# zfountas/deep-active-inference-mc

Measured on AMD Instinct MI355X. Metric: EFE rollouts/sec (64x64 dSprites, 10 MC-samples, depth 5), higher is better.
Workload: dtype f32; 1 GPU; calculate_G_repeated: 128 rows (32 roots x 4 actions) x depth 5 x 10 MC samples per GPU (BASELINE configs[1]) + action posterior; rows_per_gpu=128, samples=10, depth=5, parallelism=episodes sharded x1, weights replicated

## Files before the change

### deep-active-inference-mc_amd/csrc/decoder.hip

```cpp
#include <utility>
#include "mfma_pipe.h"

namespace efe {

template <class F, int... I> __device__ __forceinline__ void static_for_(F&& f, std::integer_sequence<int, I...>) { (f(std::integral_constant<int, I>{}), ...); }
template <int N, class F> __device__ __forceinline__ void static_for(F&& f) { static_for_(f, std::make_integer_sequence<int, N>{}); }

__host__ __device__ constexpr int w3_nch(int G) { return G == 4 ? 5 : 4; }
__host__ __device__ constexpr int w3_prod(int G, int c) {
    return G < 4 ? 5 * ((G >> 1) + 2 * (c >> 1)) + (G & 1) + 2 * (c & 1)
         : G == 4 ? (c < 2 ? 5 * (1 + 2 * c) + 4 : c < 4 ? 20 + 1 + 2 * (c - 2) : 24)
                  : (c < 2 ? 5 * (2 * c) + 4 : 20 + 2 * (c - 2));
}
__host__ __device__ constexpr bool w3_direct(int pp) { return f22_o1(pp / 5) < 0 && f22_o1(pp % 5) < 0; }
__host__ __device__ constexpr int w3_view(int pp) { return 3 * f22_view(pp / 5) + f22_view(pp % 5); }
__host__ __device__ constexpr int w3_mat(int pp) { return 4 * f22_wt(pp / 5) + f22_wt(pp % 5); }
__host__ __device__ constexpr bool w3_hits(int pp, int o) {
    const int r = o >> 2, c = o & 3, pr = pp / 5, pc = pp % 5;
    return (r == f22_o0(pr) || r == f22_o1(pr)) && (c == f22_o0(pc) || c == f22_o1(pc));
}
__host__ __device__ constexpr bool w3_seen(int G, int c, int o) {
    for (int g = 0; g < G; ++g)
        for (int k = 0; k < w3_nch(g); ++k) if (w3_hits(w3_prod(g, k), o)) return true;
    if (!w3_direct(w3_prod(G, c)))
        for (int k = 0; k < w3_nch(G); ++k)
            if ((w3_direct(w3_prod(G, k)) || k < c) && w3_hits(w3_prod(G, k), o)) return true;
    return false;
}
__host__ __device__ constexpr bool w3_uses_view(int G, int vi) {
    for (int k = 0; k < w3_nch(G); ++k) if (w3_view(w3_prod(G, k)) == vi) return true;
    return false;
}
__host__ __device__ constexpr bool f22_in(int a, int r) { return a == 0 ? r <= 1 : (a == 1 ? r == 1 : r >= 1); }
__host__ __device__ constexpr bool w3_reads(int G, int r, int c) {
    for (int vi = 0; vi < 9; ++vi) if (w3_uses_view(G, vi) && f22_in(vi / 3, r) && f22_in(vi % 3, c)) return true;
    return false;
}

constexpr int DA_PS = 17;
constexpr int DA_BIAS = 273 * DA_PS;

__host__ __device__ constexpr int wino_i0(int a) { return a == 0 ? 0 : (a == 2 ? 2 : 1); }
__host__ __device__ constexpr int wino_i1(int a) { return a == 0 ? 2 : (a == 1 ? 2 : (a == 2 ? 1 : 3)); }
__host__ __device__ constexpr float wino_s1(int a) { return a == 1 ? 1.0f : -1.0f; }
__host__ __device__ constexpr float wino_at(int r, int a) { return r == 0 ? (a < 3 ? 1.0f : 0.0f) : (a == 0 ? 0.0f : (a == 1 ? 1.0f : -1.0f)); }

template <int NR, int R0, class Pix>
__device__ __forceinline__ void wino_l1(f32x16 (&out)[NR][2], const float4* __restrict__ U, const float4* sm, const int h,
                                        const int mt_, Pix pix) {
    constexpr int PD = 4;
    const unsigned ln = (threadIdx.x & 63u) * 16u;
    const __amdgpu_buffer_rsrc_t ur = wrsrc(U);
    int mt = mt_; asm volatile("" : "+s"(mt));
    constexpr int a_lo = NR == 2 ? 0 : R0, a_hi = NR == 2 ? 4 : R0 + 3;
    auto ufrag = [&](int a, int b, int kc) { return wfrag(ur, ln, (size_t)(((4 * a + b) * 2 + mt) * 8 + kc) * 64); };
    auto bases = [&](int a, int b, int (&pb)[4]) {
        const int i0 = wino_i0(a), i1 = wino_i1(a), j0 = wino_i0(b), j1 = wino_i1(b);
        pb[0] = pix(i0, j0); pb[1] = pix(i0, j1); pb[2] = pix(i1, j0); pb[3] = pix(i1, j1);
    };
    float4 aq[PD], raw[4];
    int pb[4];
#pragma unroll
    for (int p = 0; p < PD; ++p) aq[p] = ufrag(a_lo, 0, p);
    bases(a_lo, 0, pb);
#pragma unroll
    for (int q = 0; q < 4; ++q) raw[q] = sm[pb[q] + h];
    f32x16 xacc;
    const f32x16 zero = {};
    auto otrans = [&](int a, int b, const f32x16& m, auto mask) {
        constexpr int MASK = decltype(mask)::value;
#pragma unroll
        for (int r = 0; r < NR; ++r) {
            if (!((MASK >> r) & 1)) continue;
            const float car = wino_at(R0 + r, a);
#pragma unroll
            for (int c = 0; c < 2; ++c) {
                const float cbc = wino_at(c, b);
                if (cbc == 0.0f) continue;
                const float cf = car * cbc;
#pragma unroll
                for (int e = 0; e < 16; ++e) out[r][c][e] = __builtin_fmaf(cf, m[e], out[r][c][e]);
            }
        }
    };
    auto xi_row = [&](int a, auto mask) {
        const float s1 = wino_s1(a);
        const int an = a + 1 < a_hi ? a + 1 : a;
#pragma unroll
        for (int b = 0; b < 4; ++b) {
            const float t1 = wino_s1(b);
#pragma unroll
            for (int kc = 0; kc < 8; ++kc) {
                const float4 av = aq[kc % PD];
                aq[kc % PD] = (b * 8 + kc + PD < 32) ? ufrag(a, (b * 8 + kc + PD) >> 3, (kc + PD) & 7) : ufrag(an, 0, (kc + PD) & 7);
                float4 v;
                {
                    const float4 c0 = make_float4(__builtin_fmaf(s1, raw[2].x, raw[0].x), __builtin_fmaf(s1, raw[2].y, raw[0].y),
                                                  __builtin_fmaf(s1, raw[2].z, raw[0].z), __builtin_fmaf(s1, raw[2].w, raw[0].w));
                    const float4 c1 = make_float4(__builtin_fmaf(s1, raw[3].x, raw[1].x), __builtin_fmaf(s1, raw[3].y, raw[1].y),
                                                  __builtin_fmaf(s1, raw[3].z, raw[1].z), __builtin_fmaf(s1, raw[3].w, raw[1].w));
                    v = make_float4(__builtin_fmaf(t1, c1.x, c0.x), __builtin_fmaf(t1, c1.y, c0.y), __builtin_fmaf(t1, c1.z, c0.z), __builtin_fmaf(t1, c1.w, c0.w));
                }
                if (kc < 7) {
#pragma unroll
                    for (int q = 0; q < 4; ++q) raw[q] = sm[pb[q] + 2 * (kc + 1) + h];
                } else {
                    if (b < 3) bases(a, b + 1, pb);
                    else bases(an, 0, pb);
#pragma unroll
                    for (int q = 0; q < 4; ++q) raw[q] = sm[pb[q] + h];
                }
                __builtin_amdgcn_sched_barrier(0);
                f32x16& x = xacc;
                x = __builtin_amdgcn_mfma_f32_32x32x2f32(av.x, v.x, kc == 0 ? zero : x, 0, 0, 0);
                x = __builtin_amdgcn_mfma_f32_32x32x2f32(av.y, v.y, x, 0, 0, 0);
                x = __builtin_amdgcn_mfma_f32_32x32x2f32(av.z, v.z, x, 0, 0, 0);
                x = __builtin_amdgcn_mfma_f32_32x32x2f32(av.w, v.w, x, 0, 0, 0);
            }
            otrans(a, b, xacc, mask);
        }
    };
    if constexpr (NR == 2) {
        xi_row(0, std::integral_constant<int, 1>{});
#pragma unroll 1
        for (int a = 1; a < 3; ++a) xi_row(a, std::integral_constant<int, 3>{});
        xi_row(3, std::integral_constant<int, 2>{});
    } else {
#pragma unroll 1
        for (int a = a_lo; a < a_hi; ++a) xi_row(a, std::integral_constant<int, 1>{});
    }
}
struct F22Nb { int xb, c2[3], r2; };
__device__ __forceinline__ f32x4 f22_wfrag(const __amdgpu_buffer_rsrc_t wr, const unsigned ln, int ct, int m, int kc) {
    return __builtin_bit_cast(f32x4, wfrag(wr, ln + (unsigned)kc * 1024u, (size_t)(m * 4 + ct) * 256));
}
constexpr int F22_PD = 2;
__device__ __forceinline__ void f22_l2_first(f32x4 (&aq)[F22_PD][5], const __amdgpu_buffer_rsrc_t wr, const int dn, const unsigned ln) {
    static_for<F22_PD>([&](auto p) {
        static_for<w3_nch(p >> 2)>([&](auto c) { aq[p][c] = f22_wfrag(wr, ln, dn, w3_mat(w3_prod(p >> 2, c)), p & 3); });
    });
}
__device__ __forceinline__ void f22_l2(f32x4 (&acc)[16], f32x4 (&aq)[F22_PD][5], const __amdgpu_buffer_rsrc_t wr, const int dn,
                                       const unsigned ln, const f32x4 bias4, const f32x4* smv, const F22Nb& nb) {
    constexpr int NST = 24;
    auto px = [&](int i, int jj, int kc) -> f32x4 {
        return smv[(jj == 2 ? nb.c2[i] : (i == 2 ? nb.r2 + jj * DA_PS : nb.xb + (16 * i + jj) * DA_PS)) + 4 * kc];
    };
    auto view = [&](const f32x4 (&x)[9], int vi) -> f32x4 {
        const int va = vi / 3, vb = vi % 3;
        auto cv = [&](int i) -> f32x4 { return vb == 0 ? x[3 * i] - x[3 * i + 1] : (vb == 1 ? x[3 * i + 1] : x[3 * i + 2] - x[3 * i + 1]); };
        return va == 0 ? cv(0) - cv(1) : (va == 1 ? cv(1) : cv(2) - cv(1));
    };
    const f32x4 zero4 = {};
    f32x4 tq[5], xr[9];
    static_for<9>([&](auto i) { if constexpr (w3_reads(0, i / 3, i % 3)) xr[i] = px(i / 3, i % 3, 0); });
    static_for<NST>([&](auto stc) {
        constexpr int ST = decltype(stc)::value, G = ST >> 2, KC = ST & 3, GN = (ST + 1) >> 2, KN = (ST + 1) & 3;
        constexpr int SP = (ST + F22_PD) % NST, GP = SP >> 2, KP = SP & 3;
        f32x4 vw[9], ac[5];
        static_for<9>([&](auto vi) { if constexpr (w3_uses_view(G, vi)) vw[vi] = view(xr, vi); });
#pragma unroll
        for (int c = 0; c < 5; ++c) ac[c] = aq[ST % F22_PD][c];
        static_for<w3_nch(GP)>([&](auto c) { aq[ST % F22_PD][c] = f22_wfrag(wr, ln, ST + F22_PD < NST ? 0 : dn, w3_mat(w3_prod(GP, c)), KP); });
        if constexpr (ST + 1 < NST)
            static_for<9>([&](auto i) { if constexpr (w3_reads(GN, i / 3, i % 3)) xr[i] = px(i / 3, i % 3, KN); });
        __builtin_amdgcn_sched_barrier(0);
#pragma unroll
        for (int e = 0; e < 4; ++e)
            static_for<w3_nch(G)>([&](auto c) {
                constexpr int PP = w3_prod(G, c);
                const float b = vw[w3_view(PP)][e], av = ac[c][e];
                if constexpr (w3_direct(PP)) {
                    constexpr int O = 4 * f22_o0(PP / 5) + f22_o0(PP % 5);
                    constexpr bool FIRST = KC == 0 && !w3_seen(G, c, O);
                    acc[O] = __builtin_amdgcn_mfma_f32_16x16x4f32(av, b, (FIRST && e == 0) ? bias4 : acc[O], 0, 0, 0);
                } else {
                    tq[c] = __builtin_amdgcn_mfma_f32_16x16x4f32(av, b, (KC == 0 && e == 0) ? zero4 : tq[c], 0, 0, 0);
                }
            });
        if constexpr (KC == 3)
            static_for<w3_nch(G)>([&](auto c) {
                constexpr int PP = w3_prod(G, c);
                if constexpr (!w3_direct(PP))
                    static_for<16>([&](auto o) {
                        if constexpr (w3_hits(PP, o)) {
                            if constexpr (w3_seen(G, c, o)) acc[o] = acc[o] + tq[c];
                            else acc[o] = bias4 + tq[c];
                        }
                    });
            });
    });
}
__device__ __forceinline__ void f22_l2_store(f32x4 (&acc)[16], const __amdgpu_buffer_rsrc_t yr, const unsigned yoff, const int ct, const bool on) {
#pragma unroll
    for (int orow = 0; orow < 4; ++orow)
#pragma unroll
        for (int c = 0; c < 2; ++c) {
            u32x4 lo, hi;
#pragma unroll
            for (int e = 0; e < 4; ++e) {
                const unsigned x0 = __builtin_bit_cast(unsigned, relu_bits(acc[4 * orow + c][e]));
                const unsigned x1 = __builtin_bit_cast(unsigned, relu_bits(acc[4 * orow + c + 2][e]));
                const auto sw = __builtin_amdgcn_permlane32_swap(x0, x1, false, false);
                lo[e] = sw[0]; hi[e] = sw[1];
            }
            const unsigned so = (unsigned)(((2 * (orow & 1) + c) * 4096 + 2 * ct * 512 + (orow >> 1) * 32) * 16);
            if (on) {
                __builtin_amdgcn_raw_buffer_store_b128(lo, yr, yoff, so, 0);
                __builtin_amdgcn_raw_buffer_store_b128(hi, yr, yoff, so + 512u * 16u, 0);
            }
        }
}

__global__ void __launch_bounds__(256, 2) k_dec_a(const DecAArgs a) {
    constexpr int NTHR = 256;
    constexpr int NPH = 2048 / NTHR;
    constexpr int NPE = 8;
    extern __shared__ __attribute__((aligned(16))) float4 sm[];
    const int tid = threadIdx.x;
    const int lane = tid & 63;
    const int w = __builtin_amdgcn_readfirstlane(tid >> 6);

    const float4* W1 = reinterpret_cast<const float4*>(a.w1);
    const float4* W2 = reinterpret_cast<const float4*>(a.w2);

    if ((int)blockIdx.x >= a.rows) return;
    int* const slot = reinterpret_cast<int*>(sm + DA_BIAS + 32);
    if (tid == 0) slot[0] = 2 * (int)gridDim.x + atomicAdd(a.queue, 1);
    int nimg = (int)blockIdx.x + (int)gridDim.x;
    f32x4 pf[2 * NPH];
    f32x4* smv = reinterpret_cast<f32x4*>(sm);
    {
        const f32x4* X = reinterpret_cast<const f32x4*>(a.x4) + (size_t)blockIdx.x * 4096;
#pragma unroll
        for (int it = 0; it < 2 * NPH; ++it) pf[it] = X[w * 1024 + it * 64 + lane];
    }
    for (int i = tid; i < 17 * DA_PS; i += NTHR) sm[256 * DA_PS + i] = make_float4(0.f, 0.f, 0.f, 0.f);
    if (tid < 16) sm[DA_BIAS + tid] = reinterpret_cast<const float4*>(a.b1)[tid];
    else if (tid < 32) sm[DA_BIAS + tid] = reinterpret_cast<const float4*>(a.b2)[tid - 16];

    for (int img = blockIdx.x; img < a.rows;) {
        int tl_ = tid; asm volatile("" : "+v"(tl_));
        const int j = tl_ & 31, h = (tl_ >> 5) & 1;
        const bool live = row_live(a.live, img);
        if (live) {
            const int sbase = (64 * w + ((tl_ >> 4) & 3)) * DA_PS + (tl_ & 15);
#pragma unroll
            for (int it = 0; it < 2 * NPH; ++it) smv[sbase + it * 4 * DA_PS] = pf[it];
        }
        __syncthreads();
        const int nnimg = slot[0];
        int ticket = 0;
        if (tid == 0) ticket = 2 * (int)gridDim.x + atomicAdd(a.queue, 1);
        const int l1mt = w >> 1, l1n = 32 * (w & 1) + j;
        const int l1y = 2 * (l1n >> 3) - 1, l1x = 2 * (l1n & 7) - 1;
        if (live) {
            f32x16 l1o[2][2];
#pragma unroll
            for (int g4 = 0; g4 < 4; ++g4) {
                const float4 bb = sm[DA_BIAS + l1mt * 8 + 2 * g4 + h];
#pragma unroll
                for (int rc = 0; rc < 4; ++rc) { l1o[rc >> 1][rc & 1][4 * g4] = bb.x; l1o[rc >> 1][rc & 1][4 * g4 + 1] = bb.y; l1o[rc >> 1][rc & 1][4 * g4 + 2] = bb.z; l1o[rc >> 1][rc & 1][4 * g4 + 3] = bb.w; }
            }
            wino_l1<2, 0>(l1o, W1, sm, h, l1mt, [&](int i, int jj) {
                const int y = l1y + i, x = l1x + jj;
                return ((unsigned)y < 16u && (unsigned)x < 16u ? y * 16 + x : 256) * DA_PS;
            });
            __syncthreads();
            if (tid == 0) slot[0] = ticket;
#pragma unroll
            for (int rc = 0; rc < 4; ++rc) {
                const int pix = (l1y + 1 + (rc >> 1)) * 16 + l1x + 1 + (rc & 1);
#pragma unroll
                for (int g4 = 0; g4 < 4; ++g4) {
                    const f32x16& o = l1o[rc >> 1][rc & 1];
                    float4 v;
                    v.x = relu_bits(o[4 * g4 + 0]); v.y = relu_bits(o[4 * g4 + 1]);
                    v.z = relu_bits(o[4 * g4 + 2]); v.w = relu_bits(o[4 * g4 + 3]);
                    sm[pix * DA_PS + l1mt * 8 + 2 * g4 + h] = v;
                }
            }
        } else {
            __syncthreads();
            if (tid == 0) slot[0] = ticket;
        }
        __syncthreads();
        {
            int t2_ = tid; asm volatile("" : "+v"(t2_));
            const int n = t2_ & 15, g = (t2_ >> 4) & 3;
            const int bu = 2 * w + (n >> 3), bv = n & 7;
            const int zq = 256 * DA_PS + g;
            F22Nb nb;
            nb.xb = (32 * bu + 2 * bv) * DA_PS + g;
            nb.c2[0] = bv == 7 ? zq : nb.xb + 2 * DA_PS;
            nb.c2[1] = bv == 7 ? zq : nb.xb + 18 * DA_PS;
            nb.c2[2] = bv == 7 ? zq : nb.xb + 34 * DA_PS;
            nb.r2 = nb.xb + 32 * DA_PS;
            const unsigned ln = (unsigned)(t2_ & 63) * 16u;
            const unsigned yoff = (unsigned)(((32 * bu + 2 * bv + (g >> 1)) * 2 + (g & 1)) * 16);
            const __amdgpu_buffer_rsrc_t yr = wrsrc(a.y2 + (size_t)__builtin_amdgcn_readfirstlane(img) * (32 * 32 * 64));
            auto load_next = [&](const int lo, const int hi) {
                const int pimg = __builtin_amdgcn_readfirstlane(nimg < a.rows ? nimg : img);
                const __amdgpu_buffer_rsrc_t xr = wrsrc(a.x4 + (size_t)pimg * 16384);
#pragma unroll
                for (int it = 0; it < 2 * NPH; ++it)
                    if (it >= lo && it < hi) pf[it] = __builtin_bit_cast(f32x4, wfrag(xr, (unsigned)(w * 16384 + (t2_ & 63) * 16 + (it & 3) * 1024), (size_t)(it >> 2) * 256));
            };
            if (live) {
                f32x4 aq[F22_PD][5], acc2[16];
                f22_l2_first(aq, wrsrc(W2), 0, ln);
                load_next(0, NPE);
#pragma unroll 1
                for (int ct = 0; ct < 4; ++ct) {
                    const f32x4 bias4 = smv[DA_BIAS + 16 + 4 * ct + g];
                    f22_l2(acc2, aq, wrsrc(W2 + ct * 256), ct < 3 ? 1 : 0, ln, bias4, smv, nb);
                    if (ct < 3) f22_l2_store(acc2, yr, yoff, ct, true);
                }
                load_next(NPE, 2 * NPH);
                f22_l2_store(acc2, yr, yoff, 3, true);
            } else {
                load_next(0, 2 * NPH);
            }
        }
        __syncthreads();
        img = nimg; nimg = nnimg;
    }
}

constexpr int DAS_IN = 6 * 16;
constexpr int DAS_L1 = 4 * 16;
constexpr int DAS_BIAS = (DAS_IN + 1 + DAS_L1 + 2) * DA_PS;
constexpr size_t DAS_LDS_BYTES = (DAS_BIAS + 32) * sizeof(float4);
__global__ void __launch_bounds__(256, 2) k_dec_a_s(const DecAArgs a) {
    extern __shared__ __attribute__((aligned(16))) float4 sm[];
    float4* sin = sm;
    float4* sl1 = sm + (DAS_IN + 1) * DA_PS;
    const int tid = threadIdx.x, lane = tid & 63;
    const int w = __builtin_amdgcn_readfirstlane(tid >> 6);
    const int j = lane & 31, h = lane >> 5;
    const int img = blockIdx.x >> 3, p = blockIdx.x & 7;
    if (!row_live(a.live, img)) return;
    const float4* W1 = reinterpret_cast<const float4*>(a.w1);
    const float4* W2 = reinterpret_cast<const float4*>(a.w2);
    {
        const float4* X = reinterpret_cast<const float4*>(a.x4) + (size_t)img * 4096;
        const int c4 = tid & 15, px0 = tid >> 4;
        float4 v[6];
#pragma unroll
        for (int it = 0; it < 6; ++it) {
            const int pix = px0 + 16 * it, lr = pix >> 4, y = 2 * p - 1 + lr;
            v[it] = (y >= 0 && y < 16) ? X[(y * 16 + (pix & 15)) * 16 + c4] : make_float4(0.f, 0.f, 0.f, 0.f);
        }
#pragma unroll
        for (int it = 0; it < 6; ++it) sin[(px0 + 16 * it) * DA_PS + c4] = v[it];
    }
    if (tid < 16) sin[DAS_IN * DA_PS + tid] = make_float4(0.f, 0.f, 0.f, 0.f);
    if (tid < 2 * DA_PS) sl1[DAS_L1 * DA_PS + tid] = make_float4(0.f, 0.f, 0.f, 0.f);
    if (tid < 16) sm[DAS_BIAS + tid] = reinterpret_cast<const float4*>(a.b1)[tid];
    else if (tid < 32) sm[DAS_BIAS + tid] = reinterpret_cast<const float4*>(a.b2)[tid - 16];
    __syncthreads();
    const int mt = w >> 1;
    {
        const int r = w & 1, n = j & 15;
        const int ly = 2 * (n >> 3) - 1, lx = 2 * (n & 7) - 1;
        f32x16 o[1][2];
#pragma unroll
        for (int g4 = 0; g4 < 4; ++g4) {
            const float4 bb = sm[DAS_BIAS + mt * 8 + 2 * g4 + h];
#pragma unroll
            for (int c = 0; c < 2; ++c) { o[0][c][4 * g4] = bb.x; o[0][c][4 * g4 + 1] = bb.y; o[0][c][4 * g4 + 2] = bb.z; o[0][c][4 * g4 + 3] = bb.w; }
        }
        auto pix = [&](int i, int jj) {
            const int sy = ly + 1 + i, x = lx + jj, y = 2 * p - 1 + sy;
            return ((unsigned)y < 16u && (unsigned)x < 16u ? sy * 16 + x : DAS_IN) * DA_PS;
        };
        if (r) wino_l1<1, 1>(o, W1, sin, h, mt, pix);
        else wino_l1<1, 0>(o, W1, sin, h, mt, pix);
        if (j < 16)
#pragma unroll
        for (int c = 0; c < 2; ++c)
#pragma unroll
            for (int g4 = 0; g4 < 4; ++g4) {
                float4 v;
                v.x = relu_bits(o[0][c][4 * g4 + 0]); v.y = relu_bits(o[0][c][4 * g4 + 1]);
                v.z = relu_bits(o[0][c][4 * g4 + 2]); v.w = relu_bits(o[0][c][4 * g4 + 3]);
                sl1[((ly + 1 + r) * 16 + lx + 1 + c) * DA_PS + mt * 8 + 2 * g4 + h] = v;
            }
    }
    __syncthreads();
    {
        const int n = lane & 15, g = lane >> 4, bv = n & 7;
        const int zq = DAS_L1 * DA_PS + g;
        F22Nb nb;
        nb.xb = 2 * bv * DA_PS + g;
        nb.c2[0] = bv == 7 ? zq : nb.xb + 2 * DA_PS;
        nb.c2[1] = bv == 7 ? zq : nb.xb + 18 * DA_PS;
        nb.c2[2] = (bv == 7 || p == 7) ? zq : nb.xb + 34 * DA_PS;
        nb.r2 = p == 7 ? zq : nb.xb + 32 * DA_PS;
        const unsigned ln = (unsigned)lane * 16u;
        const unsigned yoff = (unsigned)(((32 * p + 2 * bv + (g >> 1)) * 2 + (g & 1)) * 16);
        const __amdgpu_buffer_rsrc_t yr = wrsrc(a.y2 + (size_t)img * (32 * 32 * 64));
        const __amdgpu_buffer_rsrc_t wr = wrsrc(W2 + w * 256);
        f32x4 aq[F22_PD][5], acc2[16];
        f22_l2_first(aq, wr, 0, ln);
        const f32x4 bias4 = reinterpret_cast<const f32x4*>(sm)[DAS_BIAS + 16 + 4 * w + g];
        f22_l2(acc2, aq, wr, 0, ln, bias4, reinterpret_cast<const f32x4*>(sl1), nb);
        f22_l2_store(acc2, yr, yoff, w, n < 8);
    }
}

constexpr size_t DA_LDS_BYTES = (DA_BIAS + 33) * sizeof(float4);
int init_dec_b_kernels();
int init_decoder_kernels() {
    if (hipFuncSetAttribute((const void*)k_dec_a, hipFuncAttributeMaxDynamicSharedMemorySize, DA_LDS_BYTES) != hipSuccess) return 1;
    if (hipFuncSetAttribute((const void*)k_dec_a_s, hipFuncAttributeMaxDynamicSharedMemorySize, DAS_LDS_BYTES) != hipSuccess) return 1;
    return init_dec_b_kernels();
}

void launch_dec_a(const DecAArgs& a, hipStream_t st) {
    if (a.parts == 8) {
        hipLaunchKernelGGL(k_dec_a_s, dim3(a.rows * 8), dim3(256), DAS_LDS_BYTES, st, a);
        return;
    }
    const size_t lds = DA_LDS_BYTES;
    const int grid = a.rows < 512 ? a.rows : 512;
    hipLaunchKernelGGL(k_dec_a, dim3(grid), dim3(256), lds, st, a);
}


template <int PARTS>
__global__ void __launch_bounds__(256, 2) k_dec_b4(const DecBArgs a) {
    constexpr int SR = 4, NW = 4, NTHR = 256;
    constexpr int DB_RP = 33;
    constexpr int DB_PS = 17;
    constexpr int DB_IN_F4 = (SR + 1) * DB_RP * DB_PS;
    constexpr int DB_YROWS = 4 * SR + 2;
    constexpr int NPF = (SR + 1) * 512 / NTHR;
    constexpr int NS = 32 / SR;
    constexpr int NST = 24;
    extern __shared__ __attribute__((aligned(16))) float4 sm[];
    float* sH = reinterpret_cast<float*>(sm + DB_IN_F4);
    __shared__ float4 sb3[8];
    const int tid = threadIdx.x;
    const int lane = tid & 63;
    const int w = __builtin_amdgcn_readfirstlane(tid >> 6);
    const int g = lane >> 4, v = lane & 15;
    const int u = w >> 1, hf = w & 1;
    constexpr int parts = PARTS;
    const int img = parts == 1 ? (int)blockIdx.x : (int)(blockIdx.x >> 2);
    const int qtr = parts == 1 ? 0 : (int)(blockIdx.x & 3);
    if (!row_live(a.live, img)) return;
    const int s_lo = parts == 1 ? 0 : (qtr ? 2 * qtr - 1 : 0);
    const int s_hi = parts == 1 ? NS : 2 * qtr + 2;

    const int mg = a.m0 + img;
    const int gi = mg / a.rows_per_group;
    const int r = mg - gi * a.rows_per_group;
    int gt, gp, gs;
    group_decode(a.gm, gi, gt, gp, gs);
    const int mode = (gp == 0 && a.reward0) ? 1 : 0;
    const int slot = (gp == 0 && a.store0) ? gt * a.gm.S + gs : -1;
    float* po = (slot >= 0) ? a.po + ((size_t)slot * a.rows_per_group + r) * 4096 : nullptr;

    __shared__ float sq[4 * NTHR];
    __shared__ float sQ[4];
    if (tid < 8) sb3[tid] = reinterpret_cast<const float4*>(a.b3)[tid];
    if (tid < (SR + 1) * 16) sm[((tid >> 4) * DB_RP + 32) * DB_PS + (tid & 15)] = make_float4(0.f, 0.f, 0.f, 0.f);
    f32x4 w4a;
    {
        const int kh = v >> 2, kw = v & 3;
#pragma unroll
        for (int rr = 0; rr < 4; ++rr) w4a[rr] = (kh < 3 && kw < 3) ? a.w4[(3 * kh + kw) * 32 + 16 * hf + 4 * g + rr] : 0.f;
    }

    const __amdgpu_buffer_rsrc_t xr = __builtin_amdgcn_make_buffer_rsrc(const_cast<float*>(a.y2) + (size_t)img * (32 * 32 * 64), 0, 32 * 32 * 64 * 4, 0x00020000);
    const __amdgpu_buffer_rsrc_t wr = wrsrc(a.w3 + (size_t)hf * 4 * 64 * 4);
    const unsigned ln = (unsigned)lane * 16u;
    auto wf = [&](int m, int kc) -> f32x4 { return __builtin_bit_cast(f32x4, wfrag(wr, ln, (size_t)(m * 8 + kc) * 64)); };
    const float D1 = 1.00001f, D0 = 0.00001f;
    float part = 0.f;
    f32x4 pf[NPF];
    f32x4* smv = reinterpret_cast<f32x4*>(sm);
    auto prefetch = [&](int sn, int tl) {
        const unsigned lo = (unsigned)(((tl >> 5) * 512 + (tl & 31)) * 16);
        const unsigned lh = lo | (sn == NS - 1 ? 0x80000000u : 0u);
#pragma unroll
        for (int it = 0; it < NPF; ++it) {
            const int rl = it >> 1;
            const unsigned pc = (unsigned)((((rl & 1) * 16 + (it & 1) * 8) * 512 + (rl >> 1) * 32) * 16);
            pf[it] = __builtin_bit_cast(f32x4, __builtin_amdgcn_raw_buffer_load_b128(xr, rl == SR ? lh : lo, pc + (unsigned)sn * 1024u, 0));
        }
    };
    prefetch(s_lo, tid);

    const int xb = (2 * u * DB_RP + 2 * v) * DB_PS + g;
    auto px = [&](int i, int jj, int kc) -> f32x4 { return smv[xb + (i * DB_RP + jj) * DB_PS + 4 * kc]; };
    auto view = [&](const f32x4 (&x)[9], int vi) -> f32x4 {
        const int va = vi / 3, vb = vi % 3;
        auto cv = [&](int i) -> f32x4 { return vb == 0 ? sub4(x[3 * i], x[3 * i + 1]) : (vb == 1 ? x[3 * i + 1] : sub4(x[3 * i + 2], x[3 * i + 1])); };
        return va == 0 ? sub4(cv(0), cv(1)) : (va == 1 ? cv(1) : sub4(cv(2), cv(1)));
    };

    constexpr int RWG = 2 * SR / NW;
    float gh[RWG][6], gpr[RWG];
    auto g_load = [&](int oh, int q, int r0y, int hb0) {
#pragma unroll
        for (int kh = 0; kh < 3; ++kh) {
            const int tr = oh + 1 - kh;
            const bool rv = tr >= 0 && tr <= 63;
            int hs = hb0 + (tr - r0y);
            hs = hs < 0 ? hs + DB_YROWS : hs;
            hs = hs >= DB_YROWS ? hs - DB_YROWS : hs;
            hs = rv ? hs : 0;
            const float* hq = sH + ((hs * 2) * 3 + kh) * 64 + lane;
            gh[q][2 * kh] = hq[0]; gh[q][2 * kh + 1] = hq[3 * 64];
        }
    };
    auto g_sig = [&](int oh, int q) {
        float val = a.b4;
#pragma unroll
        for (int kh = 0; kh < 3; ++kh) {
            const int tr = oh + 1 - kh;
            val = add1(val, (tr >= 0 && tr <= 63) ? add1(gh[q][2 * kh], gh[q][2 * kh + 1]) : 0.f);
        }
        gpr[q] = hw_sigmoid(val);
    };
    auto g_term = [&](int oh, int q) {
#pragma clang fp contract(off)
        const float pr = gpr[q];
        const float l1 = hw_log(D1 - pr), l0 = hw_log(D0 + pr);
        const float te = __builtin_fmaf(pr - 1.0f, l1, -(pr * l0));
        const float tw = reward_term(pr, oh, lane, 64, 64, a.reward_intent);
        const float t = mode == 0 ? te : tw;
        part += oh >= 0 ? t : 0.0f;
    };
    auto g_store = [&](int oh, int q) {
        if (po && oh >= 0) {
            int owl = lane; asm volatile("" : "+v"(owl));
            (po + oh * 64)[owl] = gpr[q];
        }
    };

    auto fold = [&](int k) { sq[k * NTHR + tid] = part; part = 0.f; };
    float* const sHw = sH + g * 64 + 4 * v;
    int hb = 0, hbp = 0;
    for (int s = s_lo; s < s_hi; ++s) {
        int tl = tid; asm volatile("" : "+v"(tl));
        const bool gq = parts == 1 ? true : s == 2 * qtr + 1;
        const int oh0 = 2 * SR * (s - 1) - 1 + w, oh1 = oh0 + NW;
        {
            f32x4* const sp = smv + ((tl & 31) >> 1) * (2 * DB_PS) + 2 * (tl >> 5) + (tl & 1);
#pragma unroll
            for (int it = 0; it < NPF; ++it) sp[((it >> 1) * DB_RP + (it & 1)) * DB_PS] = pf[it];
        }
        f32x4 aq[5];
#pragma unroll
        for (int c = 0; c < w3_nch(0); ++c) aq[c] = wf(w3_mat(w3_prod(0, c)), 0);
        __syncthreads();

        const f32x4 bias4 = __builtin_bit_cast(f32x4, sb3[4 * hf + g]);
        const f32x4 zero4 = {};
        f32x4 acc[16], tq[5];
        f32x4 xr[9];
        static_for<9>([&](auto i) { if constexpr (w3_reads(0, i / 3, i % 3)) xr[i] = px(i / 3, i % 3, 0); });
        static_for<NST>([&](auto stc) {
            constexpr int ST = decltype(stc)::value, G = ST >> 2, KC = ST & 3, GN = (ST + 1) >> 2, KN = (ST + 1) & 3;
            f32x4 vw[9], ac[5];
            static_for<9>([&](auto vi) { if constexpr (w3_uses_view(G, vi)) vw[vi] = view(xr, vi); });
#pragma unroll
            for (int c = 0; c < 5; ++c) ac[c] = aq[c];
            if constexpr (ST + 1 < NST) {
                static_for<w3_nch(GN)>([&](auto c) { aq[c] = wf(w3_mat(w3_prod(GN, c)), KN); });
                static_for<9>([&](auto i) { if constexpr (w3_reads(GN, i / 3, i % 3)) xr[i] = px(i / 3, i % 3, KN); });
            }
            __builtin_amdgcn_sched_barrier(0);
#pragma unroll
            for (int e = 0; e < 4; ++e)
                static_for<w3_nch(G)>([&](auto c) {
                    constexpr int PP = w3_prod(G, c);
                    const float b = vw[w3_view(PP)][e], av = ac[c][e];
                    if constexpr (w3_direct(PP)) {
                        constexpr int O = 4 * f22_o0(PP / 5) + f22_o0(PP % 5);
                        constexpr bool FIRST = KC == 0 && !w3_seen(G, c, O);
                        acc[O] = __builtin_amdgcn_mfma_f32_16x16x4f32(av, b, (FIRST && e == 0) ? bias4 : acc[O], 0, 0, 0);
                    } else {
                        tq[c] = __builtin_amdgcn_mfma_f32_16x16x4f32(av, b, (KC == 0 && e == 0) ? zero4 : tq[c], 0, 0, 0);
                    }
                });
            if constexpr (KC == 3)
                static_for<w3_nch(G)>([&](auto c) {
                    constexpr int PP = w3_prod(G, c);
                    if constexpr (!w3_direct(PP))
                        static_for<16>([&](auto o) {
                            if constexpr (w3_hits(PP, o)) {
                                if constexpr (w3_seen(G, c, o)) acc[o] = add4(acc[o], tq[c]);
                                else acc[o] = add4(bias4, tq[c]);
                            }
                        });
                });
            if (gq) {
                if constexpr (ST == 0) { g_load(oh0, 0, 2 * SR * (s - 1), hbp); g_load(oh1, 1, 2 * SR * (s - 1), hbp); }
                if constexpr (ST == 2) g_sig(oh0, 0);
                if constexpr (ST == 5) g_term(oh0, 0);
                if constexpr (ST == 8) g_sig(oh1, 1);
                if constexpr (ST == 11) g_term(oh1, 1);
            }
        });
        prefetch((s < NS - 1) ? s + 1 : NS - 1, tl);
#pragma unroll
        for (int orow = 0; orow < 4; ++orow) {
            f32x4 T[4];
#pragma unroll
            for (int oc = 0; oc < 4; ++oc)
#pragma unroll
                for (int e = 0; e < 4; ++e) acc[4 * orow + oc][e] = relu_bits(acc[4 * orow + oc][e]);
#pragma unroll
            for (int e = 0; e < 4; ++e)
#pragma unroll
                for (int oc = 0; oc < 4; ++oc)
                    T[oc] = __builtin_amdgcn_mfma_f32_16x16x4f32(w4a[e], acc[4 * orow + oc][e], e == 0 ? zero4 : T[oc], 0, 0, 0);
            f32x4 hv;
            hv[0] = add1(add1(T[1][0], T[0][1]), dpp_shr1_zero(T[3][2]));
            hv[1] = add1(add1(T[2][0], T[1][1]), T[0][2]);
            hv[2] = add1(add1(T[3][0], T[2][1]), T[1][2]);
            hv[3] = add1(add1(dpp_shl1_zero(T[0][0]), T[3][1]), T[2][2]);
            int hsw = hb + 4 * u + orow;
            hsw = hsw >= DB_YROWS ? hsw - DB_YROWS : hsw;
            if (g < 3) *reinterpret_cast<f32x4*>(sHw + (hsw * 2 + hf) * (3 * 64)) = hv;
        }
        __syncthreads();
        if (gq) { g_store(oh0, 0); g_store(oh1, 1); }
        if (parts == 1 && (s == 2 || s == 4 || s == 6)) fold(s / 2 - 1);
        if (s == s_hi - 1) {
#pragma unroll
            for (int q = 0; q <= RWG; ++q) {
                if (q == RWG && (w != 0 || s != NS - 1)) break;
                const int oh = 2 * SR * s - 1 + q * NW + w;
                g_load(oh, 0, 2 * SR * s, hb); g_sig(oh, 0); g_term(oh, 0); g_store(oh, 0);
            }
        }
        hbp = hb;
        hb += 2 * SR;
        hb = hb >= DB_YROWS ? hb - DB_YROWS : hb;
    }
    fold(parts == 1 ? 3 : 0);
    __syncthreads();
    if (w < (parts == 1 ? 4 : 1)) {
        const float* qk = sq + w * NTHR + lane;
        float val = add1(add1(qk[0], qk[64]), add1(qk[128], qk[192]));
#pragma unroll
        for (int o = 32; o > 0; o >>= 1) val += __shfl_xor(val, o);
        if (lane == 0) sQ[w] = val;
    }
    __syncthreads();
    if (tid == 0) {
        if (parts == 1) a.val[mg] = add1(add1(sQ[0], sQ[1]), add1(sQ[2], sQ[3]));
        else a.valq[(size_t)mg * 4 + qtr] = sQ[0];
    }
}

constexpr size_t DB_LDS4D = ((5 * 33) * 17) * sizeof(float4) + 18 * 2 * 3 * 64 * sizeof(float);
int init_dec_b_kernels() {
    if (hipFuncSetAttribute((const void*)k_dec_b4<1>, hipFuncAttributeMaxDynamicSharedMemorySize, DB_LDS4D) != hipSuccess) return 1;
    if (hipFuncSetAttribute((const void*)k_dec_b4<4>, hipFuncAttributeMaxDynamicSharedMemorySize, DB_LDS4D) != hipSuccess) return 1;
    return 0;
}

void launch_dec_b(const DecBArgs& a, hipStream_t st) {
    if (a.parts == 4) hipLaunchKernelGGL(k_dec_b4<4>, dim3(a.rows * 4), dim3(256), DB_LDS4D, st, a);
    else hipLaunchKernelGGL(k_dec_b4<1>, dim3(a.rows), dim3(256), DB_LDS4D, st, a);
}

__host__ __device__ inline int fc4_spg(int mtiles) { return ((mtiles + 7) / 8 + 7) / 8; }
template <int NT>
__global__ void __launch_bounds__(256, 2) k_fc4(const GemmArgs a) {
    constexpr int RT = 32 * NT;
    extern __shared__ __attribute__((aligned(16))) float4 sm[];
    const int tid = threadIdx.x;
    const int lane = tid & 63;
    const int w = __builtin_amdgcn_readfirstlane(tid >> 6);
    const int j = lane & 31, h = lane >> 5;
    const int fgrp = blockIdx.x & 7;
    const int nper = gridDim.x >> 3, k = blockIdx.x >> 3;
    const int SPG = fc4_spg(a.mtiles);
    const int nsteps = ((a.n_pix + RT - 1) / RT) * SPG;
    const int q0 = (int)(((long)nsteps * k) / nper), q1 = (int)(((long)nsteps * (k + 1)) / nper);
    f32x4* smv = reinterpret_cast<f32x4*>(sm);
    const float4* Wl = reinterpret_cast<const float4*>(a.Wp);
    auto xaddr = [&](int t, int (&bs)[NT], int (&sw)[NT], int& wt) {
        wt = t;
#pragma unroll
        for (int nt = 0; nt < NT; ++nt) { bs[nt] = (nt * 32 + j) * 64 + t * 16; sw[nt] = j & 15; }
    };
    int cur_rt = -1;
    uint32_t krow[2] = {0, 0}, kstream[2] = {0, 0}, kstage[2] = {0, 0};
    bool rv[2] = {false, false};
#pragma unroll 1
    for (int q = q0; q < q1; ++q) {
        const int rt = q / SPG, fs = q - rt * SPG;
        const int row0 = rt * RT;
        if (rt != cur_rt) {
            if (cur_rt >= 0) __syncthreads();
            cur_rt = rt;
            const f32x4* X = reinterpret_cast<const f32x4*>(a.X);
#pragma unroll
            for (int it = 0; it < 8 * NT; ++it) {
                const int idx = it * 256 + tid;
                const int r = idx >> 6, c4 = idx & 63;
                const int gr = row0 + r;
                smv[r * 64 + (c4 ^ (r & 15))] = (gr < a.n_pix) ? X[(size_t)gr * 64 + c4] : (f32x4)(0.f);
            }
            __syncthreads();
#pragma unroll
            for (int nt = 0; nt < NT; ++nt) {
                const int m = row0 + nt * 32 + j;
                rv[nt] = m < a.n_pix;
                const int mg = a.m0 + (rv[nt] ? m : 0);
                const int g = mg / a.rows_per_group;
                krow[nt] = global_row(a.gm.ids, a.gm.ids_div, mg - g * a.rows_per_group, a.row_offset);
                const uint2 key = group_key(a.gm, g);
                kstream[nt] = key.x; kstage[nt] = key.y;
            }
        }
        const int mt0 = (fgrp * SPG + fs) * 8 + 2 * w;
        if (mt0 >= a.mtiles) continue;
        f32x16 acc[2][NT];
#pragma unroll
        for (int mt = 0; mt < 2; ++mt)
#pragma unroll
            for (int nt = 0; nt < NT; ++nt)
#pragma unroll
                for (int e = 0; e < 16; ++e) acc[mt][nt][e] = 0.f;
        float4 bq[2][4];
#pragma unroll
        for (int mt = 0; mt < 2; ++mt)
#pragma unroll
            for (int g4 = 0; g4 < 4; ++g4) bq[mt][g4] = *reinterpret_cast<const float4*>(a.bias + (mt0 + mt) * 32 + 8 * g4 + 4 * h);
        tap_loop<2, NT>(acc, 4, Wl, sm, h, xaddr, DenseWIdx{mt0});
#pragma unroll
        for (int nt = 0; nt < NT; ++nt) {
            if (!rv[nt]) continue;
            const uint4 rnd = noise_words(a.k0, a.k1, a.tag, (uint32_t)((mt0 * 32) >> 7), krow[nt], kstream[nt], kstage[nt]);
            float* yp = a.Y + (size_t)(row0 + nt * 32 + j) * a.ldy;
#pragma unroll
            for (int mt = 0; mt < 2; ++mt)
#pragma unroll
                for (int g4 = 0; g4 < 4; ++g4) {
                    const int co = (mt0 + mt) * 32 + 8 * g4 + 4 * h;
                    const float4 bb = bq[mt][g4];
                    const uint32_t word = ((co >> 5) & 3) == 0 ? rnd.x : ((co >> 5) & 3) == 1 ? rnd.y : ((co >> 5) & 3) == 2 ? rnd.z : rnd.w;
                    float v[4] = {acc[mt][nt][4 * g4 + 0] + bb.x, acc[mt][nt][4 * g4 + 1] + bb.y,
                                  acc[mt][nt][4 * g4 + 2] + bb.z, acc[mt][nt][4 * g4 + 3] + bb.w};
#pragma unroll
                    for (int e = 0; e < 4; ++e) v[e] = ((word >> ((co + e) & 31)) & 1u) ? fmaxf(v[e], 0.f) * 2.0f : 0.0f;
                    *reinterpret_cast<float4*>(yp + co) = make_float4(v[0], v[1], v[2], v[3]);
                }
        }
    }
}

void launch_fc4(const GemmArgs& a, hipStream_t st) {
    if (a.n_pix <= 32) {
        const int nsteps = fc4_spg(a.mtiles);
        hipLaunchKernelGGL(k_fc4<1>, dim3(8 * (nsteps < 64 ? nsteps : 64)), dim3(256), 32 * 64 * sizeof(float4), st, a);
        return;
    }
    const int nsteps = ((a.n_pix + 63) / 64) * fc4_spg(a.mtiles);
    const int nper = nsteps < 64 ? nsteps : 64;
    hipLaunchKernelGGL(k_fc4<2>, dim3(8 * nper), dim3(256), 64 * 64 * sizeof(float4), st, a);
}

}
```

Before: 11770 rollouts/s.

## Deepen layer-3 MFMA software pipeline and interleave epilogue work with sched groups

Double-buffers the weight fragments and input reads two stages ahead instead of one, and computes views one stage early. The partial-sum adds for indirect products are spread across the following group's stages instead of being bunched at the last K-chunk. The sigmoid, log and term epilogue work is split into finer pieces spread over more stages. Explicit sched_group_barrier sequences interleave the MFMAs with VALU and memory ops. The aim is to hide load latency and keep the matrix pipe busy, at the cost of more live registers and the risk of lower occupancy or spills.

```diff
diff --git a/deep-active-inference-mc_amd/csrc/decoder.hip b/deep-active-inference-mc_amd/csrc/decoder.hip
--- a/deep-active-inference-mc_amd/csrc/decoder.hip
+++ b/deep-active-inference-mc_amd/csrc/decoder.hip
@@ -31,11 +31,44 @@
     for (int k = 0; k < w3_nch(G); ++k) if (w3_view(w3_prod(G, k)) == vi) return true;
     return false;
 }
+__host__ __device__ constexpr bool w3_direct_into(int G, int o) {
+    if (G > 5) return false;
+    for (int k = 0; k < w3_nch(G); ++k) {
+        const int pp = w3_prod(G, k);
+        if (w3_direct(pp) && 4 * f22_o0(pp / 5) + f22_o0(pp % 5) == o) return true;
+    }
+    return false;
+}
+__host__ __device__ constexpr int w3_add_step(int G, int c, int o) {
+    if (w3_direct_into(G + 1, o)) return 0;
+    int n = 0, k = 0;
+    for (int cc = 0; cc < w3_nch(G); ++cc) {
+        if (w3_direct(w3_prod(G, cc))) continue;
+        for (int oo = 0; oo < 16; ++oo)
+            if (w3_hits(w3_prod(G, cc), oo) && !w3_direct_into(G + 1, oo)) { if (cc == c && oo == o) k = n; ++n; }
+    }
+    return k * 4 / n;
+}
+__host__ __device__ constexpr int w3_nadds(int G, int KC) {
+    int n = 0;
+    if (G < 0) return 0;
+    for (int c = 0; c < w3_nch(G); ++c) {
+        if (w3_direct(w3_prod(G, c))) continue;
+        for (int o = 0; o < 16; ++o) if (w3_hits(w3_prod(G, c), o) && w3_add_step(G, c, o) == KC) ++n;
+    }
+    return n;
+}
 __host__ __device__ constexpr bool f22_in(int a, int r) { return a == 0 ? r <= 1 : (a == 1 ? r == 1 : r >= 1); }
 __host__ __device__ constexpr bool w3_reads(int G, int r, int c) {
     for (int vi = 0; vi < 9; ++vi) if (w3_uses_view(G, vi) && f22_in(vi / 3, r) && f22_in(vi % 3, c)) return true;
     return false;
 }
+__host__ __device__ constexpr int w3_nreads(int G) {
+    int n = 0;
+    for (int i = 0; i < 9; ++i) n += w3_reads(G, i / 3, i % 3) ? 1 : 0;
+    return n;
+}
+__host__ __device__ constexpr int w3_nsubs(int G) { return G == 0 ? 3 : G == 1 ? 1 : G == 2 ? 1 : G == 3 ? 0 : G == 4 ? 4 : 6; }
 
 constexpr int DA_PS = 17;
 constexpr int DA_BIAS = 273 * DA_PS;
@@ -525,15 +558,19 @@
         }
         gpr[q] = hw_sigmoid(val);
     };
-    auto g_term = [&](int oh, int q) {
+    float gl1, gl0;
+    auto g_log1 = [&](int q) { gl1 = hw_log(D1 - gpr[q]); };
+    auto g_log0 = [&](int q) { gl0 = hw_log(D0 + gpr[q]); };
+    auto g_fin = [&](int oh, int q, bool on) {
 #pragma clang fp contract(off)
         const float pr = gpr[q];
-        const float l1 = hw_log(D1 - pr), l0 = hw_log(D0 + pr);
+        const float l1 = gl1, l0 = gl0;
         const float te = __builtin_fmaf(pr - 1.0f, l1, -(pr * l0));
         const float tw = reward_term(pr, oh, lane, 64, 64, a.reward_intent);
         const float t = mode == 0 ? te : tw;
-        part += oh >= 0 ? t : 0.0f;
-    };
+        part += (on && oh >= 0) ? t : 0.0f;
+    };
+    auto g_term = [&](int oh, int q) { g_log1(q); g_log0(q); g_fin(oh, q, true); };
     auto g_store = [&](int oh, int q) {
         if (po && oh >= 0) {
             int owl = lane; asm volatile("" : "+v"(owl));
@@ -553,58 +590,85 @@
 #pragma unroll
             for (int it = 0; it < NPF; ++it) sp[((it >> 1) * DB_RP + (it & 1)) * DB_PS] = pf[it];
         }
-        f32x4 aq[5];
-#pragma unroll
-        for (int c = 0; c < w3_nch(0); ++c) aq[c] = wf(w3_mat(w3_prod(0, c)), 0);
+        f32x4 aq[2][5];
+        static_for<2>([&](auto p) {
+            static_for<w3_nch(0)>([&](auto c) { aq[p][c] = wf(w3_mat(w3_prod(0, c)), p); });
+        });
         __syncthreads();
 
         const f32x4 bias4 = __builtin_bit_cast(f32x4, sb3[4 * hf + g]);
         const f32x4 zero4 = {};
-        f32x4 acc[16], tq[5];
-        f32x4 xr[9];
-        static_for<9>([&](auto i) { if constexpr (w3_reads(0, i / 3, i % 3)) xr[i] = px(i / 3, i % 3, 0); });
+        f32x4 acc[16], tq[2][5];
+        f32x4 xr2[2][9], vv[2][9];
+        auto raw_req = [&](auto sc) {
+            constexpr int S = decltype(sc)::value;
+            static_for<9>([&](auto i) { if constexpr (w3_reads(S >> 2, i / 3, i % 3)) xr2[S & 1][i] = px(i / 3, i % 3, S & 3); });
+        };
+        auto views = [&](auto sc) {
+            constexpr int S = decltype(sc)::value;
+            static_for<9>([&](auto vi) { if constexpr (w3_uses_view(S >> 2, vi)) vv[S & 1][vi] = view(xr2[S & 1], vi); });
+        };
+        raw_req(std::integral_constant<int, 0>{});
+        raw_req(std::integral_constant<int, 1>{});
+        views(std::integral_constant<int, 0>{});
         static_for<NST>([&](auto stc) {
-            constexpr int ST = decltype(stc)::value, G = ST >> 2, KC = ST & 3, GN = (ST + 1) >> 2, KN = (ST + 1) & 3;
-            f32x4 vw[9], ac[5];
-            static_for<9>([&](auto vi) { if constexpr (w3_uses_view(G, vi)) vw[vi] = view(xr, vi); });
-#pragma unroll
-            for (int c = 0; c < 5; ++c) ac[c] = aq[c];
-            if constexpr (ST + 1 < NST) {
-                static_for<w3_nch(GN)>([&](auto c) { aq[c] = wf(w3_mat(w3_prod(GN, c)), KN); });
-                static_for<9>([&](auto i) { if constexpr (w3_reads(GN, i / 3, i % 3)) xr[i] = px(i / 3, i % 3, KN); });
-            }
+            constexpr int ST = decltype(stc)::value, G = ST >> 2, KC = ST & 3, GP = (ST + 2) >> 2, KP = (ST + 2) & 3;
+            f32x4 ac[5];
+#pragma unroll
+            for (int c = 0; c < 5; ++c) ac[c] = aq[ST & 1][c];
             __builtin_amdgcn_sched_barrier(0);
+            if constexpr (ST + 2 < NST) {
+                static_for<w3_nch(GP)>([&](auto c) { aq[ST & 1][c] = wf(w3_mat(w3_prod(GP, c)), KP); });
+                raw_req(std::integral_constant<int, ST + 2>{});
+            }
+            if constexpr (G > 0)
+                static_for<w3_nch(G - 1)>([&](auto c) {
+                    constexpr int PP = w3_prod(G - 1, c);
+                    if constexpr (!w3_direct(PP))
+                        static_for<16>([&](auto o) {
+                            if constexpr (w3_hits(PP, o) && w3_add_step(G - 1, c, o) == KC) {
+                                if constexpr (w3_seen(G - 1, c, o)) acc[o] = add4(acc[o], tq[(G - 1) & 1][c]);
+                                else acc[o] = add4(bias4, tq[(G - 1) & 1][c]);
+                            }
+                        });
+                });
 #pragma unroll
             for (int e = 0; e < 4; ++e)
                 static_for<w3_nch(G)>([&](auto c) {
                     constexpr int PP = w3_prod(G, c);
-                    const float b = vw[w3_view(PP)][e], av = ac[c][e];
+                    const float b = vv[ST & 1][w3_view(PP)][e], av = ac[c][e];
                     if constexpr (w3_direct(PP)) {
                         constexpr int O = 4 * f22_o0(PP / 5) + f22_o0(PP % 5);
                         constexpr bool FIRST = KC == 0 && !w3_seen(G, c, O);
                         acc[O] = __builtin_amdgcn_mfma_f32_16x16x4f32(av, b, (FIRST && e == 0) ? bias4 : acc[O], 0, 0, 0);
                     } else {
-                        tq[c] = __builtin_amdgcn_mfma_f32_16x16x4f32(av, b, (KC == 0 && e == 0) ? zero4 : tq[c], 0, 0, 0);
+                        tq[G & 1][c] = __builtin_amdgcn_mfma_f32_16x16x4f32(av, b, (KC == 0 && e == 0) ? zero4 : tq[G & 1][c], 0, 0, 0);
                     }
                 });
-            if constexpr (KC == 3)
-                static_for<w3_nch(G)>([&](auto c) {
-                    constexpr int PP = w3_prod(G, c);
-                    if constexpr (!w3_direct(PP))
-                        static_for<16>([&](auto o) {
-                            if constexpr (w3_hits(PP, o)) {
-                                if constexpr (w3_seen(G, c, o)) acc[o] = add4(acc[o], tq[c]);
-                                else acc[o] = add4(bias4, tq[c]);
-                            }
-                        });
-                });
-            if (gq) {
-                if constexpr (ST == 0) { g_load(oh0, 0, 2 * SR * (s - 1), hbp); g_load(oh1, 1, 2 * SR * (s - 1), hbp); }
-                if constexpr (ST == 2) g_sig(oh0, 0);
-                if constexpr (ST == 5) g_term(oh0, 0);
-                if constexpr (ST == 8) g_sig(oh1, 1);
-                if constexpr (ST == 11) g_term(oh1, 1);
-            }
+            if constexpr (ST + 1 < NST) views(std::integral_constant<int, ST + 1>{});
+            if constexpr (ST == 1) g_load(oh0, 0, 2 * SR * (s - 1), hbp);
+            if constexpr (ST == 2) g_sig(oh0, 0);
+            if constexpr (ST == 3) g_load(oh1, 1, 2 * SR * (s - 1), hbp);
+            if constexpr (ST == 4) g_log1(0);
+            if constexpr (ST == 5) g_log0(0);
+            if constexpr (ST == 6) g_fin(oh0, 0, gq);
+            if constexpr (ST == 7) g_sig(oh1, 1);
+            if constexpr (ST == 8) g_log1(1);
+            if constexpr (ST == 9) g_log0(1);
+            if constexpr (ST == 10) g_fin(oh1, 1, gq);
+            constexpr int NM = 4 * w3_nch(G);
+            constexpr int NX = (ST + 1 < NST ? 4 * w3_nsubs((ST + 1) >> 2) : 0) + 4 * w3_nadds(G - 1, KC)
+                             + (ST + 2 < NST ? w3_nch(GP) + w3_nreads(GP) : 0) + (ST >= 1 && ST <= 10 ? 10 : 0);
+            constexpr int NE = (G == 5 && KC == 0) ? 4 : 0;
+            static_for<NE>([&](auto) {
+                __builtin_amdgcn_sched_group_barrier(0x002, 4, 0);
+                __builtin_amdgcn_sched_group_barrier(0x008, 1, 0);
+            });
+            static_for<NM - NE>([&](auto i) {
+                constexpr int K = ((i + 1) * (NX - 4 * NE)) / (NM - NE) - (i * (NX - 4 * NE)) / (NM - NE);
+                __builtin_amdgcn_sched_group_barrier(0x008, 1, 0);
+                if constexpr (K > 0) __builtin_amdgcn_sched_group_barrier(0x522, K, 0);
+            });
         });
         prefetch((s < NS - 1) ? s + 1 : NS - 1, tl);
 #pragma unroll
```

Measured after the change: 11800 rollouts/s (median of 3 runs). About the same (+0.3%).
